# tjiiv-cprg/EPro-PnP

Hardware: AMD Instinct MI355X
Metric: PnP instances/sec (fwd+bwd, N=512 pts, 512 samples) (higher is better)
Workload: dtype f32; 1 GPU; C2 batched synthetic: 4096 objects/GPU x N=512 points, S=512 MC samples, K=4 AMIS iters, L=3 LM iters, EProPnP6DoF fwd+bwd; objects_per_gpu=4096, objects_total=4096, num_points=512, mc_samples=512, amis_iters=4, lm_iters=3, dof=6, parallelism=objects sharded x1, no data-path collective

## Files before the change

epro-pnp_amd/csrc/amis_common.h:

```cpp
#pragma once
#include "pnp_host.h"
#include "tuning.h"

namespace pnp {

typedef PNP_FIT_T fit_t;

__device__ __forceinline__ float sat_mul(float x, float one_v) {
  return __builtin_amdgcn_fmed3f(x * one_v, 0.0f, 1.0f);
}

__device__ __forceinline__ float sat_fma(float a, float b, float c) {
  return __builtin_amdgcn_fmed3f(fmaf(a, b, c), 0.0f, 1.0f);
}

__device__ __forceinline__ float clamp_below(float x, float lo) {
  int xi, li;
  memcpy(&xi, &x, 4);
  memcpy(&li, &lo, 4);
  const int mi = max(xi, li);
  float r;
  memcpy(&r, &mi, 4);
  return r;
}
// ... 58 lines not shown


PNP_FIT_FN void fit_translation(fit_t (&C)[3][3], const float* fallback_diag, float* rec) {
  fit_t invd[3];
  const bool ok = cholesky<3, fit_t>(C, invd);
  rec[37] = ok ? 0.f : 1.f;
  if (!ok) {
#pragma unroll
    for (int i = 0; i < 3; ++i) {
#pragma unroll
      for (int j = 0; j < 3; ++j) C[i][j] = (i == j) ? (fit_t)fallback_diag[i] : fit_t(0);
      invd[i] = fit_t(1) / (fit_t)fallback_diag[i];
    }
  }
  fit_t Li[3][3];
  tri_inverse<3, fit_t>(C, invd, Li);
  float sl = 0.f;
#pragma unroll
  for (int i = 0; i < 3; ++i) {
    sl += fast_log((float)C[i][i]);
#pragma unroll
    for (int j = 0; j <= i; ++j) {
      rec[3 + tri(i, j)] = (float)C[i][j];
      rec[9 + tri(i, j)] = (float)Li[i][j];
    }
  }
  rec[15] = student_t3_log_norm(sl);
}

constexpr int kRefitMaxVals = 21;
constexpr int kRefitRedFloats = kRefitMaxVals * kSumTRow + 24;
constexpr int kRefitHalfVals = 11;
constexpr int kRefitHalfFloats = kRefitHalfVals * kSumTRow + 24;

template <int NV, int ROWS = kRefitMaxVals>
PNP_FN void wave_sum_t(float (&v)[NV], float* lds, int lane) {
  static_assert(NV <= ROWS, "scratch rows");
  float* tot = lds + ROWS * kSumTRow;
#pragma unroll
  for (int i = 0; i < NV; ++i) lds[i * kSumTRow + lane] = v[i];
  wave_lds_fence();
#pragma unroll
  for (int base = 0; base < NV; base += 16) {
    const int row = base + (lane >> 2);
    float part = 0.f;
    if (row < NV) {
      const float4* r = reinterpret_cast<const float4*>(lds + row * kSumTRow + 16 * (lane & 3));
      const float4 a = r[0], b = r[1], c = r[2], d = r[3];
      part = (((a.x + a.y) + (a.z + a.w)) + ((b.x + b.y) + (b.z + b.w))) + (((c.x + c.y) + (c.z + c.w)) + ((d.x + d.y) + (d.z + d.w)));
    }
    part = quad_sum(part);
    if (row < NV && (lane & 3) == 0) tot[row] = part;
  }
  wave_lds_fence();
#pragma unroll
  for (int i = 0; i < NV; ++i) v[i] = tot[i];
  wave_lds_fence();
}

template <int NV, int ROWS = kRefitMaxVals>
PNP_FN void refit_sum(float (&v)[NV], float* scratch, int lane) {
  wave_sum_t<NV, ROWS>(v, scratch, lane);
}

template <int NV>
PNP_FN void wave_sum_fit(fit_t (&v)[NV], float* lds, int lane) {
  static_assert(NV <= 8 && NV * 64 * sizeof(fit_t) <= kRefitHalfFloats * sizeof(float), "one row of 64 per value, eight lanes per row");
  fit_t* row = reinterpret_cast<fit_t*>(lds);
#pragma unroll
  for (int i = 0; i < NV; ++i) row[i * 64 + lane] = v[i];
  wave_lds_fence();
  if (lane < 8 * NV) {
    fit_t* r = row + 8 * lane;
    r[0] = ((r[0] + r[1]) + (r[2] + r[3])) + ((r[4] + r[5]) + (r[6] + r[7]));
  }
  wave_lds_fence();
  if (lane < NV) {
    fit_t* r = row + 64 * lane;
    r[0] = ((r[0] + r[8]) + (r[16] + r[24])) + ((r[32] + r[40]) + (r[48] + r[56]));
  }
  wave_lds_fence();
#pragma unroll
  for (int i = 0; i < NV; ++i) v[i] = row[64 * i];
  wave_lds_fence();
}

PNP_FN void refit_translation_cov(const AmisParams& a, const float* smp, const float* lgw, int S, int M, float mx, float mu0, float mu1,
                                  float mu2, float invZ, float* scratch, int lane, fit_t (&C)[6]) {
  fit_t dl[3];
#pragma unroll
  for (int i = 0; i < 6; ++i) C[i] = fit_t(0);
#pragma unroll
  for (int i = 0; i < 3; ++i) dl[i] = fit_t(0);
  if (PNP_ABLATED(a, 8)) C[0] = C[2] = C[5] = fit_t(1);
  else
  for (int m = lane; m < M; m += 64) {
    const float e = fast_exp(lgw[m] - mx);
    const fit_t d0 = (fit_t)(smp[m] - mu0), d1 = (fit_t)(smp[S + m] - mu1), d2 = (fit_t)(smp[2 * S + m] - mu2);
    const fit_t e0 = (fit_t)e * d0, e1 = (fit_t)e * d1, e2 = (fit_t)e * d2;
    dl[0] += e0; dl[1] += e1; dl[2] += e2;
    C[0] += e0 * d0; C[1] += e1 * d0; C[2] += e1 * d1;
    C[3] += e2 * d0; C[4] += e2 * d1; C[5] += e2 * d2;
  }
  if (!PNP_ABLATED(a, 16)) {
    wave_sum_fit<6>(C, scratch, lane);
    wave_sum_fit<3>(dl, scratch, lane);
  }
  const fit_t iz = (fit_t)invZ;
#pragma unroll
  for (int i = 0; i < 3; ++i) dl[i] *= iz;
#pragma unroll
  for (int i = 0; i < 3; ++i)
#pragma unroll
    for (int j = 0; j <= i; ++j) C[tri(i, j)] = C[tri(i, j)] * iz - dl[i] * dl[j];
  const fit_t tol = fit_t(1e-12);
  const fit_t l21 = C[4] - C[3] * C[1] / C[0];
  const fit_t p1 = C[2] - C[1] * C[1] / C[0];
  const fit_t p2 = C[5] - C[3] * C[3] / C[0] - l21 * l21 / p1;
  if (p1 <= tol * C[2] || p2 <= tol * C[5]) C[0] = fit_t(NAN);
}

PNP_FIT_FN void fit_factor_pair(fit_t (&A)[4][4], int which, float dispersion, const float (&fallback)[4], float* rec) {
  const fit_t m01 = A[0][0] * A[1][1] - A[0][1] * A[1][0], m02 = A[0][0] * A[1][2] - A[0][2] * A[1][0],
               m03 = A[0][0] * A[1][3] - A[0][3] * A[1][0], m12 = A[0][1] * A[1][2] - A[0][2] * A[1][1],
               m13 = A[0][1] * A[1][3] - A[0][3] * A[1][1], m23 = A[0][2] * A[1][3] - A[0][3] * A[1][2];
  const fit_t n01 = A[2][0] * A[3][1] - A[2][1] * A[3][0], n02 = A[2][0] * A[3][2] - A[2][2] * A[3][0],
               n03 = A[2][0] * A[3][3] - A[2][3] * A[3][0], n12 = A[2][1] * A[3][2] - A[2][2] * A[3][1],
               n13 = A[2][1] * A[3][3] - A[2][3] * A[3][1], n23 = A[2][2] * A[3][3] - A[2][3] * A[3][2];
  const float det = (float)(m01 * n23 - m02 * n13 + m03 * n12 + m12 * n03 - m13 * n02 + m23 * n01);
  const fit_t add = (which == 0) ? (fit_t)(sqrtf(sqrtf(det)) * dispersion) : fit_t(0);
  fit_t invd[4];
#pragma unroll
  for (int i = 0; i < 4; ++i) A[i][i] += add;
  const bool ok = cholesky<4, fit_t>(A, invd) && (add == add);
  if (!ok) {
#pragma unroll
    for (int i = 0; i < 4; ++i) {
#pragma unroll
      for (int j = 0; j < 4; ++j) A[i][j] = (i == j) ? (fit_t)fallback[i] : fit_t(0);
// ... 185 lines not shown
    if (!done && (acc || a == kVmTries - 1)) {
      x = ((u3 - 0.5f >= 0.0f) ? 2.0f : -2.0f) * atan2f(srm1 * sh, srp1 * ch);
    }
    done = done || acc;
  }
  float y = x + loc + 3.14159265358979f;
  y = y - 6.283185307179586f * floorf(y * 0.15915494309189535f);
  return y - 3.14159265358979f;
}


template <int PL>
PNP_FN void store_pose(float* dst, const float (&ps)[PL]) {
  typedef float f4_a4 __attribute__((vector_size(16), aligned(4)));
  const f4_a4 head = {ps[0], ps[1], ps[2], ps[3]};
  *reinterpret_cast<f4_a4*>(dst) = head;
  if (PL == 7) {
    const f4_a4 tail = {ps[3], ps[PL > 4 ? 4 : 0], ps[PL > 5 ? 5 : 0], ps[PL > 6 ? 6 : 0]};
    *reinterpret_cast<f4_a4*>(dst + 3) = tail;
  }
}

struct AmisCtx {
  float* ptab;
  float* smp;
  float* cst;
  float* mixl;
  float* lgw;
  float* cpart;
  float* prop;
  float* red;
  float* nzb;
  float* rred;
  int S, K, s, T, tid, b;
  int cstride;
};

template <int DOF>
PNP_FN void base_noise(const AmisParams& a, int b, int m, float (&out)[8]) {
  const uint32_t k0 = (uint32_t)a.seed, k1 = (uint32_t)(a.seed >> 32);
  const uint32_t c2 = (uint32_t)a.offset, c3base = (uint32_t)(a.offset >> 32) * 64u;
  float nrm[12];
#pragma unroll
  for (int q = 0; q < (DOF == 6 ? 3 : 2); ++q) {
    const Philox4 r = philox4x32_10((uint32_t)b, (uint32_t)m, c2, c3base + q, k0, k1);
    box_muller(r.v[0], r.v[1], nrm[q * 4], nrm[q * 4 + 1]);
    box_muller(r.v[2], r.v[3], nrm[q * 4 + 2], nrm[q * 4 + 3]);
  }
  out[0] = nrm[0]; out[1] = nrm[1]; out[2] = nrm[2];
  out[3] = nrm[3] * nrm[3] + nrm[4] * nrm[4] + nrm[5] * nrm[5];
  if (DOF == 6) {
    out[4] = nrm[6]; out[5] = nrm[7]; out[6] = nrm[8]; out[7] = nrm[9];
  } else {
    out[4] = out[5] = out[6] = out[7] = 0.f;
  }
}

template <int DOF>
PNP_FN void amis_base_noise(const AmisCtx& cx, const AmisParams& a, int it, int first) {
  if (cx.nzb == nullptr || cx.tid < first) return;
  for (int n = cx.tid - first; n < cx.s; n += cx.T - first) {
    float nz8[8];
    base_noise<DOF>(a, cx.b, it * cx.s + n, nz8);
    reinterpret_cast<float4*>(cx.nzb)[2 * n] = make_float4(nz8[0], nz8[1], nz8[2], nz8[3]);
    reinterpret_cast<float4*>(cx.nzb)[2 * n + 1] = make_float4(nz8[4], nz8[5], nz8[6], nz8[7]);
  }
}

template <int DOF>
PNP_FN void amis_draw(const AmisCtx& cx, const Problem& p, const AmisParams& a, int it, const float (&Kc)[9],
                      const float* __restrict__ noise, float* __restrict__ pose_samples, int n0 = 0, int cnt = -1) {
  constexpr int PL = PoseLen<DOF>::value;
  constexpr int NZ = (DOF == 6) ? 8 : 4 + 3 * kVmTries;
  float* ptab = cx.ptab; float* smp = cx.smp;
  const int S = cx.S, K = cx.K, s = cx.s, T = cx.T, tid = cx.tid, b = cx.b;
  const float* rec = cx.prop + it * kPropStride;
  const bool nz_aliased = (cx.nzb != nullptr) && (cx.nzb == cx.ptab);
  float4 nz_a = make_float4(0.f, 0.f, 0.f, 0.f), nz_b = nz_a;
  if (nz_aliased) {
    if (tid < s) {
      nz_a = reinterpret_cast<const float4*>(cx.nzb)[2 * tid];
      nz_b = reinterpret_cast<const float4*>(cx.nzb)[2 * tid + 1];
    }
    __syncthreads();
  }
  const int n_end = (cnt < 0) ? s : n0 + cnt;
  for (int n = n0 + tid; n < n_end; n += T) {
    const int m = it * s + n;
    float z[3], chi2, g[4];
    if (noise != nullptr) {
      const float* nz = noise + (((size_t)b * K + it) * s + n) * NZ;
      z[0] = nz[0]; z[1] = nz[1]; z[2] = nz[2]; chi2 = nz[3];
      if (DOF == 6) {
        g[0] = nz[4]; g[1] = nz[5]; g[2] = nz[6]; g[3] = nz[7];
// ... 79 lines not shown
PNP_FN void amis_weights(const AmisCtx& cx, const AmisParams& a, int it, int WP) {
  constexpr int PL = PoseLen<DOF>::value;
  float* smp = cx.smp; float* cst = cx.cst; float* mixl = cx.mixl; float* lgw = cx.lgw; float* cpart = cx.cpart; float* prop = cx.prop;
  const int S = cx.S, s = cx.s, T = cx.T, tid = cx.tid;
  const float* rec = prop + it * kPropStride;
  const int M = (it + 1) * s;
  const float log_n = logf((float)(it + 1));
  for (int m = tid; m < M; m += T) {
    float ps[PL];
#pragma unroll
    for (int i = 0; i < PL; ++i) ps[i] = smp[i * S + m];
    float mix;
    if (m >= it * s) {
      if (WP > 0) {
        float c = cpart[m - it * s];
        for (int q = 1; q < WP; ++q) c += cpart[q * cx.cstride + (m - it * s)];
        cst[m] = c;
      }
      if (PNP_ABLATED(a, 4)) {
        mix = 0.f;
      } else {
        mix = proposal_logprob<DOF>(prop, ps);
        for (int j = 1; j <= it; ++j) mix = log_add_exp(mix, proposal_logprob<DOF>(prop + j * kPropStride, ps));
      }
    } else {
      mix = PNP_ABLATED(a, 4) ? 0.f : log_add_exp(mixl[m], proposal_logprob<DOF>(rec, ps));
    }
    mixl[m] = mix;
    lgw[m] = -cst[m] - (mix - log_n);
  }

}

template <int DOF, bool HALF = false>
PNP_FN void amis_refit(const AmisCtx& cx, const AmisParams& a, int it) {
  static_assert(!HALF || DOF == 6, "the half-size scratch serves the 6-DoF refit");
  constexpr int ROWS = HALF ? kRefitHalfVals : kRefitMaxVals;
  float* smp = cx.smp; float* lgw = cx.lgw; float* prop = cx.prop; float* red = cx.red;
  const int S = cx.S, s = cx.s;
  const float* rec = prop + it * kPropStride;
  const int M = (it + 1) * s;
  float* nrec = prop + (it + 1) * kPropStride;
  if (wave_id() != 0) {
    amis_base_noise<DOF>(cx, a, it + 1, 64);
    __syncthreads();
    return;
  }
  const int T = 64, tid = cx.tid;
  PNP_REFIT_BEGIN();
  if (PNP_ABLATED(a, 2)) {
    for (int i = tid; i < kPropStride; i += T) nrec[i] = rec[i];
    __syncthreads();
    return;
  }
  float mx = -INFINITY;
  for (int m = tid; m < M; m += T) mx = fmaxf(mx, lgw[m]);
  mx = wave_max(mx);
  const float p0 = rec[0], p1 = rec[1], p2 = rec[2];
  if (DOF == 6) {
    float mom[15];
#pragma unroll
    for (int i = 0; i < 15; ++i) mom[i] = 0.f;
    if (PNP_ABLATED(a, 8)) mom[0] = mom[4] = mom[6] = mom[9] = mom[13] = mom[14] = 1.f;
    else
    for (int m = tid; m < M; m += T) {
      const float e = fast_exp(lgw[m] - mx);
      const float d0 = smp[m] - p0, d1 = smp[S + m] - p1, d2 = smp[2 * S + m] - p2;
      mom[0] += e;
      mom[1] += e * d0; mom[2] += e * d1; mom[3] += e * d2;
// ... 50 lines not shown
          red[10 + i] = (float)invd[i];
#pragma unroll
          for (int j = 0; j < i; ++j) red[tri(i, j)] = (float)Sg[i][j];
        }
      }
      wave_lds_fence();
#pragma unroll
      for (int i = 0; i < 10; ++i) Lf[i] = red[i];
#pragma unroll
      for (int i = 0; i < 4; ++i) Ld[i] = red[10 + i];
      wave_lds_fence();
#pragma unroll
      for (int i = 0; i < 11; ++i) acc[i] = 0.f;
      for (int m = tid; m < M; m += T) {
        const float e = fast_exp(lgw[m] - mx);
        const float q0 = smp[3 * S + m], q1 = smp[4 * S + m], q2 = smp[5 * S + m], q3 = smp[6 * S + m];
        const float y0 = q0 * Ld[0];
        const float y1 = fmaf(-Lf[tri(1, 0)], y0, q1) * Ld[1];
        const float y2 = fmaf(-Lf[tri(2, 1)], y1, fmaf(-Lf[tri(2, 0)], y0, q2)) * Ld[2];
        const float y3 = fmaf(-Lf[tri(3, 2)], y2, fmaf(-Lf[tri(3, 1)], y1, fmaf(-Lf[tri(3, 0)], y0, q3))) * Ld[3];
        const float Mq = fmaf(y3, y3, fmaf(y2, y2, fmaf(y1, y1, y0 * y0)));
        const float iw = e * fast_rcp(fmaxf(Mq, a.eps));
        acc[10] += iw;
        acc[0] += iw * q0 * q0;
        acc[1] += iw * q1 * q0; acc[2] += iw * q1 * q1;
        acc[3] += iw * q2 * q0; acc[4] += iw * q2 * q1; acc[5] += iw * q2 * q2;
        acc[6] += iw * q3 * q0; acc[7] += iw * q3 * q1; acc[8] += iw * q3 * q2; acc[9] += iw * q3 * q3;
      }
      refit_sum<11, ROWS>(acc, cx.rred, tid);
    }
    PNP_REFIT_PHASE(1);
    if (tid < 2) {
      if (tid == 0) {
        nrec[0] = mu0; nrec[1] = mu1; nrec[2] = mu2;
        nrec[39] = 0.f;
      }
      fit_t A4[4][4];
      const fit_t inorm = (a.mle_iter > 0) ? fit_t(1) / (fit_t)acc[10] : fit_t(0);
#pragma unroll
      for (int i = 0; i < 4; ++i)
#pragma unroll
        for (int j = 0; j <= i; ++j) {
          fit_t v = (a.mle_iter > 0) ? (fit_t)acc[tri(i, j)] * inorm + ((i == j) ? (fit_t)a.eps : fit_t(0))
                                      : ((i == j) ? fit_t(1) : fit_t(0));
          if (tid == 1) v = (i < 3) ? c6[tri(i, j)] : ((i == j) ? fit_t(1) : fit_t(0));
          A4[i][j] = v;
          A4[j][i] = v;
        }
      const float dflt[4] = {1.f, 1.f, 1.f, 1.f};
      fit_factor_pair(A4, tid, a.dispersion, dflt, nrec);
    }
    PNP_REFIT_PHASE(2);
  } else {
    float mom[6];
#pragma unroll
    for (int i = 0; i < 6; ++i) mom[i] = 0.f;
    for (int m = tid; m < M; m += T) {
      const float e = fast_exp(lgw[m] - mx);
      const float d0 = smp[m] - p0, d1 = smp[S + m] - p1, d2 = smp[2 * S + m] - p2;
      mom[0] += e;
      mom[1] += e * d0; mom[2] += e * d1; mom[3] += e * d2;
      const float yaw = smp[3 * S + m];
      float sy, cy;
      sincos_rad(yaw, sy, cy);
      mom[4] += e * sy;
      mom[5] += e * cy;
    }
// ... 34 lines not shown
```

epro-pnp_amd/csrc/amis_forward_mfma.hip:

```cpp
#include "amis_common.h"
#include "dispatch.h"

namespace pnp {



template <bool BOUNDS, bool FOLDED = false>
__device__ __forceinline__ void huber_cost_4(const floatx4& hx, const floatx4& hy, const floatx4& hz, const float4& w4,
                                             float zmin_v, float one_v, const Bounds& bd, f32x2 (&acc2)[2]) {
  static_assert(!(BOUNDS && FOLDED), "the clamp acts on the un-weighted projection");
  const f32x2 wu2 = {w4.x, w4.x}, wv2 = {w4.y, w4.y}, cu2 = {w4.z, w4.z}, cv2 = {w4.w, w4.w};
  const f32x2 mhalf = {-0.5f, -0.5f};
#pragma unroll
  for (int h = 0; h < 2; ++h) {
    const float z0 = clamp_below(hz[2 * h], zmin_v), z1 = clamp_below(hz[2 * h + 1], zmin_v);
    const f32x2 rz2 = {fast_rcp(z0), fast_rcp(z1)};
    const f32x2 hx2 = {hx[2 * h], hx[2 * h + 1]}, hy2 = {hy[2 * h], hy[2 * h + 1]};
    f32x2 rx2, ry2;
    if (FOLDED) {
      rx2 = fma2(hx2, rz2, cu2);
      ry2 = fma2(hy2, rz2, cv2);
    } else {
      f32x2 px2 = hx2 * rz2, py2 = hy2 * rz2;
      if (BOUNDS) {
        px2 = f32x2{clamp_lu(px2[0], bd.lbx, bd.ubx), clamp_lu(px2[1], bd.lbx, bd.ubx)};
        py2 = f32x2{clamp_lu(py2[0], bd.lby, bd.uby), clamp_lu(py2[1], bd.lby, bd.uby)};
      }
      rx2 = fma2(px2, wu2, cu2);
      ry2 = fma2(py2, wv2, cv2);
    }
    const f32x2 s2 = fma2(rx2, rx2, ry2 * ry2);
    const f32x2 rho2 = {fast_sqrt(s2[0]), fast_sqrt(s2[1])};
    const f32x2 m2 = {sat_mul(rho2[0], one_v), sat_mul(rho2[1], one_v)};
    acc2[h] = fma2(m2, fma2(mhalf, m2, rho2), acc2[h]);
  }
}

constexpr int kChunk = 1024;

struct MfmaShape {
  int chunk;
  int s16;
  int ahead;
  int chunks;
};

template <int DOF, bool BOUNDS, int NPT, bool SPILL = false, bool SPLIT = false, bool BF16 = false, bool CHUNKED = false, bool WLDS = false>
__global__ __launch_bounds__(512, SPLIT ? 2 : (DOF == 6 ? (NPT <= 8 ? (BF16 ? (WLDS ? PNP_FWD_WLDS_MINW : PNP_FWD_BF16_MINW) : PNP_FWD_MINW) : 2) : (NPT <= 2 ? 3 : 2))) void amis_forward_mfma_kernel(Problem p, AmisParams a_in, MfmaShape sh,
                                                                  const float* __restrict__ pose_opt,
                                                                  const float* __restrict__ pose_cov,
                                                                  const float* __restrict__ noise,
                                                                  float* __restrict__ pose_samples,
                                                                  float* __restrict__ logweights,
                                                                  float* __restrict__ proposals,
                                                                  float* __restrict__ spill, int nsplit,
                                                                  float* __restrict__ xch) {
  static_assert(!SPILL || NPT == 0, "the spill variant streams the points");
  static_assert(!SPLIT || NPT > 0, "the split over workgroups is a register-mode variant");
  static_assert(!WLDS || (BF16 && DOF == 6 && NPT > 0 && !SPLIT && !CHUNKED && !SPILL), "weights in LDS: the one-workgroup bf16 6-DoF kernel");
  constexpr int PL = PoseLen<DOF>::value;
  const int G = SPLIT ? nsplit : 1;
  static_assert(!CHUNKED || (NPT > 0 && !SPLIT && !SPILL), "chunks are a register-mode variant of the one-workgroup kernel");
  const int CH = CHUNKED ? sh.chunks : 1;
  const int GT = SPLIT ? G : CH;
  int b, part = 0;
  if (SPLIT) {
    const int g = (int)blockIdx.x, per = (p.B + 7) >> 3, idx = g >> 3;
    part = idx % G;
    b = (g & 7) * per + idx / G;
  } else {
    b = object_of_block(p.B);
  }
  if (b >= p.B) return;
  AmisParams a = a_in;
  if (a.offset_dev != nullptr) a.offset += *a.offset_dev;
  const int T = (int)blockDim.x, tid = (int)threadIdx.x, lane = lane_id(), wv = wave_id(), W = T >> 6;
  const int S = a.S, K = a.K, s = S / K, s16 = sh.s16, NC = sh.chunk;

  PNP_PHASES_BEGIN(6);
  PNP_DYN_SMEM(float, smem);
  constexpr bool kRegs = NPT > 0;
  static_assert(!BF16 || NPT > 0, "the split projection is a register-mode variant");
  constexpr bool kBf = BF16;
  typedef ProjOp<kBf> Proj;
  constexpr bool kFold = kRegs && !BOUNDS && !kBf;
  const int WPs = kRegs ? (G > 1 ? G : W) : 1;
  const int cpart_rows = kRegs ? (SPLIT ? W + G : W) : 1;
  float* ptab = smem;
  float* pB = ptab + 12 * s16;
  float* pW = pB + 4 * NC;
  float* smp = SPILL ? spill + (size_t)b * (PL + 3) * S : pW + 4 * NC;
  float* cst = smp + PL * S;
  float* mixl = cst + S;
  float* lgw = mixl + S;
  float* cpart = SPILL ? pW + 4 * NC : smp + (((PL + 3) * S + 3) & ~3);
  float* gath = cpart + W * s16;
  float* prop = cpart + (WLDS ? max(cpart_rows * s16, kRefitHalfFloats) : cpart_rows * s16) + (SPLIT ? 4 : 0);
  float* red = prop + K * kPropStride;
  float* wl = red + 256;
  float* rred = WLDS ? cpart : red + 256;
  float* nzb = (s <= T) ? ptab : (WLDS ? wl + W * NPT * 64 : rred + kRefitRedFloats);

  float Kc[9], delta;
  Bounds bd;
  load_camera<BOUNDS>(p, b, Kc, bd, delta);
  const float zmin_v = to_vgpr(p.z_min), one_v = to_vgpr(1.0f);
  const HuberScale hs = huber_scale(delta);
  const float inv_delta = hs.inv_delta, delta_sq = hs.delta_sq;

  const bool tiled = SPILL && s > s16;
  AmisCtx cx;
  cx.ptab = ptab; cx.smp = smp; cx.cst = cst; cx.mixl = mixl; cx.lgw = lgw; cx.cpart = SPLIT ? gath : cpart; cx.prop = prop; cx.red = red;
  cx.S = S; cx.K = K; cx.s = s; cx.T = T; cx.tid = tid; cx.b = b; cx.cstride = s16;
  cx.nzb = (noise == nullptr && W > 1 && sh.ahead) ? nzb : nullptr;
  cx.rred = rred;

  if (!tiled)
    for (int i = tid; i < 12 * (s16 - s); i += T) ptab[12 * s + i] = 0.f;
  if (tid < (DOF == 6 ? 2 : 1))
    initial_fit<DOF>(pose_opt + (size_t)b * PL, pose_cov + (size_t)b * DOF * DOF, a.eps, a.dispersion, prop, tid);
  if (part == 0 && tid == T - 1) denormalise_pose_opt<DOF>(a, pose_opt, b);
  const int nchunk = kRegs ? 1 : (p.N + NC - 1) / NC;
  auto load_chunk = [&](int c0) {
    const int cnt = min(NC, ((p.N - c0 + 15) >> 4) << 4);
    for (int n = tid; n < cnt; n += T) {
      const Point q = load_point(p, b, c0 + n);
      reinterpret_cast<float4*>(pB)[n] = make_float4(q.X, q.Y, q.Z, 1.0f);
      const float wu = q.wu * inv_delta, wv = q.wv * inv_delta;
      reinterpret_cast<float4*>(pW)[n] = make_float4(wu, wv, -q.u * wu, -q.v * wv);
    }
  };
  typename Proj::T rB[kRegs ? NPT : 1];
  float4 rW[kRegs ? NPT : 1];
  auto load_tiles = [&](int pt) {
#pragma unroll
    for (int i = 0; i < (kRegs ? NPT : 1); ++i) {
      const Point q = load_point(p, b, ((pt * W + wv) + GT * W * i) * 16 + (lane & 15));
      const int k4 = lane >> 4;
      const int wslot = (wv * NPT + i) * 16 + (lane & 15);
      const float bval = (k4 == 0) ? q.X : (k4 == 1) ? q.Y : (k4 == 2) ? q.Z : 1.0f;
      rB[i] = Proj::b(bval);
      const float wu = q.wu * inv_delta, wv = q.wv * inv_delta;
      if constexpr (WLDS) {
        if (k4 == 0) reinterpret_cast<float4*>(wl)[wslot] = make_float4(wu, wv, -q.u * wu, -q.v * wv);
      } else {
        rW[i] = kFold ? make_float4(bval * wu, bval * wv, -q.u * wu, -q.v * wv) : make_float4(wu, wv, -q.u * wu, -q.v * wv);
      }
    }
// ... 142 lines not shown
        const unsigned v = xwg_poll(slot + q * s16 + m, (((miss | gone_parts) >> q) & 1u) ? 0u : a.split_timeout);
        if (v == kXwgEmpty) miss |= 1u << q; else gath[q * s16 + m] = bits_f32(v);
      }
      if (miss) atomicOr(reinterpret_cast<int*>(missw), (int)miss);
      __syncthreads();
      unsigned todo = *missw;
      gone_parts |= todo;
      if (todo) {
        if (tid == 0) raise_status(p, EPROPNP_ST_SPLIT_TIMEOUT, b);
        for (int q = 0; q < G; ++q) {
          if (!((todo >> q) & 1u)) continue;
          load_tiles(q);
          sweep_regs();
          __syncthreads();
          for (int m = tid; m < s; m += T) {
            float c = cpart[m];
            for (int w = 1; w < W; ++w) c += cpart[w * s16 + m];
            gath[q * s16 + m] = bits_f32(xwg_payload(c));
          }
          __syncthreads();
        }
        load_tiles(part);
      }
    }
    PNP_PHASE(2);

    if (tiled) __syncthreads();
    AmisCtx cxw = cx;
    cxw.tid = (int)f32_bits(to_vgpr(bits_f32((unsigned)tid)));
    amis_weights<DOF>(cxw, a, it, tiled ? 0 : WPs);
    __syncthreads();
    PNP_PHASE(3);
    if (it == K - 1) break;
    amis_refit<DOF, WLDS>(cxw, a, it);
    PNP_PHASE(4);
  }

  if (part == 0) {
    int st_bits = 0;
    for (int m = tid; m < S; m += T) {
      const float lw = lgw[m];
      logweights[(size_t)m * p.B + b] = lw;
      if (a.sample_costs != nullptr) a.sample_costs[(size_t)m * p.B + b] = cst[m];
      st_bits |= (lw == lw && lw != INFINITY) ? 0 : EPROPNP_ST_NONFINITE_WEIGHT;
    }
    for (int i = tid; i < K; i += T)
      st_bits |= (prop[i * kPropStride + 37] != 0.f || prop[i * kPropStride + 38] != 0.f) ? EPROPNP_ST_CHOL_FALLBACK : 0;
    raise_status(p, st_bits, b);
  }
  if (proposals != nullptr && part == 0)
    for (int i = tid; i < K * kPropStride; i += T) proposals[(size_t)b * K * kPropStride + i] = prop[i];
  PNP_PHASE(5);
  advance_counters(a, p.B * G);
  PNP_PHASES_FLUSH(6);
}

int tuning_phase_cycles(unsigned long long* out, int reset) { return tuning::read_cycles(out, reset, true); }

template <class F>
static int dispatch_npt(int npt, F&& f) {
  switch (npt) {
    case 0: return f(ic<0>{});
    case 1: return f(ic<1>{});
    case 2: return f(ic<2>{});
    case 4: return f(ic<4>{});
    case 8: return f(ic<8>{});
    case 12: return f(ic<12>{});
    default: return f(ic<16>{});
  }
}

static int forward_split_parts(int B, int ptiles) {
  const long wgs = padded_object_grid(B), cus = device_cu_count();
  int g = 8;
  while (g > 1 && (wgs * g > cus || 8 * g > ptiles)) g >>= 1;
  if (g < 4) g = 1;
  { int ov[1]; if (env_ints("EPROPNP_FWD_SPLIT", ov, 1) && (ov[0] == 1 || ov[0] == 2 || ov[0] == 4 || ov[0] == 8) && wgs * ov[0] <= 4096 && 4 * ov[0] <= ptiles) g = ov[0]; }
  return g;
}

unsigned long long amis_forward_split_bytes(const epropnp_problem* prob, int mc_samples, int num_iter) {
  if (prob == nullptr || prob->num_obj <= 0 || num_iter <= 0 || mc_samples % num_iter != 0) return 0;
  const int ptiles = (prob->num_pts + 15) / 16;
  const int g = forward_split_parts(prob->num_obj, ptiles);
  if (g <= 1 || (ptiles + 4 * g - 1) / (4 * g) > 8) return 0;
  const int s16 = ((mc_samples / num_iter + 15) / 16) * 16;
  return sizeof(float) * (unsigned long long)prob->num_obj * num_iter * g * s16;
}

struct FwdPlan {
  MfmaShape sh;
  int waves, npt, G;
  size_t smem;
  bool bf16, spilled, truncated, chunked;
  bool wlds;
};

constexpr size_t kLdsPerCu = 160 * 1024, kLdsGranule = 1280;

static int plan_amis_forward(const epropnp_problem* prob, int S, int K, unsigned long long scratch_bytes, FwdPlan* out) {
  const int B = prob->num_obj, N = prob->num_pts;
  const int s = S / K;
  const int PL = prob->dof == 6 ? 7 : 4;
  MfmaShape& sh = out->sh;
  sh.s16 = ((s + 15) / 16) * 16;
  const int ptiles = (N + 15) / 16;
  const int npt_opts[6] = {1, 2, 4, 8, 12, 16};
  int waves = 4, npt = 0, best = 1 << 30;
  for (int w : {4, 8, 2, 1}) {
    for (int o : npt_opts) {
      if (w * o >= ptiles && w * o < best) { best = w * o; waves = w; npt = o; }
      if (w * o >= ptiles) break;
    }
  }
  if (prob->dof == 4 && npt >= 12) npt = 0;
  if (B < 512 && waves == 4 && npt == 8) { waves = 8; npt = 4; }
  { int ov[2]; if (tune_ints("fwd_mfma", ov, 2) && (ov[0] == 1 || ov[0] == 2 || ov[0] == 4 || ov[0] == 8) && (ov[1] == 0 || ov[1] == 1 || ov[1] == 2 || ov[1] == 4 || ov[1] == 8 || ov[1] == 12 || ov[1] == 16) && (ov[1] == 0 || ov[0] * ov[1] >= ptiles)) { waves = ov[0]; npt = ov[1]; } }
  if (npt == 0) {
    sh.chunk = ((N + 15) / 16) * 16;
    if (sh.chunk > kChunk) sh.chunk = kChunk;
    if (best == (1 << 30)) waves = 4;
    const int tiles = sh.s16 / 16;
    while (waves > 1 && waves > tiles) waves /= 2;
  } else {
    sh.chunk = 0;
  }
  int G = 1;
  {
    const int g = forward_split_parts(B, ptiles);
// ... 29 lines not shown
    spilled = true;
    waves = 8; npt = 0; G = 1; sh.chunks = 1;
    sh.chunk = ((N + 15) / 16) * 16;
    if (sh.chunk > kChunk) sh.chunk = kChunk;
    const int tiles = sh.s16 / 16;
    while (waves > 1 && waves > tiles) waves /= 2;
    smem = lds_bytes(true);
    if (smem > 160 * 1024) {
      sh.ahead = 0;
      const size_t fixed = sizeof(float) * (8 * (size_t)sh.chunk + (size_t)K * kPropStride + 256 + kRefitRedFloats);
      const size_t rows = (160 * 1024 - fixed) / (sizeof(float) * 13);
      if ((size_t)sh.s16 > rows) sh.s16 = (int)(rows / 16) * 16;
      if (sh.s16 < 16) return fail(EPROPNP_EINVAL, "amis_forward: no LDS left for a pose tile (%d points per chunk)", sh.chunk);
      smem = lds_bytes(true);
    }
  }
  bool bf16 = npt >= 1;
  if (const char* e = getenv("EPROPNP_FWD_PROJ")) bf16 = (e[0] == 'f') ? false : bf16;
  out->waves = waves; out->npt = npt; out->G = G; out->smem = smem;
  out->bf16 = bf16; out->spilled = spilled; out->truncated = sh.s16 < s16_full;
  out->chunked = !spilled && G == 1 && npt == 8 && (sh.chunks > 1 || (bf16 && tune_flag("fwd_chunked")));
  out->wlds = false;
  if (prob->dof == 6 && bf16 && !spilled && !out->chunked && G == 1 && waves == 4 && npt == 8) {
    const size_t smem_w = lds_bytes(false, true);
    const size_t granules = (smem_w + kLdsGranule - 1) / kLdsGranule * kLdsGranule;
    bool take = 4 * granules <= kLdsPerCu && (long)padded_object_grid(B) > 3L * device_cu_count();
    { int ov[1]; if (tune_ints("fwd_wlds", ov, 1)) take = ov[0] != 0 && smem_w <= kLdsPerCu; }
    if (take) { out->wlds = true; out->smem = smem_w; }
    if (take && PNP_FWD_WLDS_MINW < 4) {
      const size_t hold = kLdsPerCu / PNP_FWD_WLDS_MINW / kLdsGranule * kLdsGranule;
      if (out->smem < hold) out->smem = hold;
    }
  }
  return EPROPNP_OK;
}

int plan_amis_forward_record(const epropnp_problem* prob, int S, int K, unsigned long long scratch_bytes, int32_t* out) {
  FwdPlan plan;
  if (int rc = plan_amis_forward(prob, S, K, scratch_bytes, &plan)) return rc;
  out[0] = plan.waves; out[1] = plan.npt; out[2] = plan.G; out[3] = plan.sh.chunks; out[4] = plan.bf16; out[5] = plan.spilled;
  out[6] = plan.truncated; out[7] = plan.chunked;
  return EPROPNP_OK;
}

int launch_amis_forward(const epropnp_problem* prob, const epropnp_amis_params* am, const float* pose_opt,
                        const float* pose_cov, const float* noise, float* pose_samples, float* logweights,
                        float* proposals, hipStream_t st, const DenormOut* dn, float* sample_costs) {
  if (int rc = check_problem(prob)) return rc;
  if (!am) return fail(EPROPNP_EINVAL, "amis_forward: params NULL");
  if (am->num_iter <= 0 || am->mc_samples <= 0 || am->mc_samples % am->num_iter != 0)
    return fail(EPROPNP_EINVAL, "amis_forward: mc_samples (%d) must be a positive multiple of num_iter (%d)",
                am->mc_samples, am->num_iter);
  if (prob->num_obj == 0) return EPROPNP_OK;
  if (!pose_opt || !pose_cov || !pose_samples || !logweights) return fail(EPROPNP_EINVAL, "amis_forward: NULL pointer");
  const Problem d = to_device_problem(prob);
  const int S = am->mc_samples, K = am->num_iter;
  const int PL = prob->dof == 6 ? 7 : 4;
  FwdPlan plan;
  if (int rc = plan_amis_forward(prob, S, K, am->split_scratch != nullptr ? am->split_scratch_bytes : 0, &plan)) return rc;
  const MfmaShape sh = plan.sh;
  const int waves = plan.waves, npt = plan.npt, G = plan.G;
  const size_t smem = plan.smem;
  const bool bf16 = plan.bf16;
  AmisParams k;
  k.S = S; k.K = K; k.unused_wp = 1; k.eps = am->eps; k.mle_iter = am->acg_mle_iter; k.dispersion = am->acg_dispersion;
  k.seed = am->seed; k.offset = am->offset; k.offset_dev = (const unsigned long long*)am->offset_dev; k.ablate = 0;
  k.advance = (am->advance && am->advance_ticket && am->advance_count > 0) ? (unsigned long long*)am->advance : nullptr;
  k.advance_ticket = (int*)am->advance_ticket; k.advance_count = am->advance_count;
  k.split_timeout = split_timeout_cycles();
  k.dn_offset = dn ? dn->offset : nullptr; k.dn_samples = dn ? dn->samples : nullptr; k.dn_pose_opt = dn ? dn->pose_opt : nullptr;
  k.sample_costs = sample_costs;
  { int ab[1]; if (tune_ints("ablate", ab, 1)) k.ablate = ab[0]; }
  float* spill = nullptr;
  if (plan.spilled &&
      hipMallocAsync((void**)&spill, sizeof(float) * (size_t)(PL + 3) * S * d.B, st) != hipSuccess) {
    (void)hipGetLastError();
    return fail(EPROPNP_ELAUNCH, "amis_forward: mc_samples %d needs a %zu B scratch buffer and hipMallocAsync failed "
                "(stream capture?)", S, sizeof(float) * (size_t)(PL + 3) * S * d.B);
  }
  const dim3 grid(padded_object_grid(d.B)), block(64 * waves);
  if (spill != nullptr) {
    dispatch_dof_bounds(prob->dof, has_bounds(prob), [&](auto DOF, auto BND) -> int {
      auto kern = amis_forward_mfma_kernel<decltype(DOF)::value, decltype(BND)::value, 0, true>;
      allow_dynamic_lds((const void*)kern, smem);
      PNP_LAUNCH(kern, grid, block, smem, st, d, k, sh, pose_opt, pose_cov, noise, pose_samples, logweights, proposals, spill, 1,
                 (float*)nullptr);
      return 0;
    });
    const int rc = check_launch("amis_forward_mfma_kernel (sampler state in global scratch)");
    (void)hipFreeAsync(spill, st);
    return rc;
  }
  float* xch = nullptr;
  char* owned = nullptr;
  dim3 grid_split = grid;
  if (G > 1) {
    const size_t xbytes = sizeof(float) * (size_t)d.B * K * G * sh.s16;
    char* mem = (am->split_scratch != nullptr && am->split_scratch_bytes >= xbytes) ? (char*)am->split_scratch : nullptr;
    if (mem == nullptr) {
      if (hipMallocAsync((void**)&mem, xbytes, st) != hipSuccess) {
        (void)hipGetLastError();
        return fail(EPROPNP_ELAUNCH, "amis_forward: scratch for the %d-way split (%zu B) could not be allocated", G, xbytes);
      }
      owned = mem;
    }
    if (!exchange_prefilled(mem, xbytes) &&
        launch_fill_u32(mem, 0xffffffffu, xbytes / 4, st) != EPROPNP_OK) {
      (void)hipGetLastError();
      return fail(EPROPNP_ELAUNCH, "amis_forward: could not fill the split scratch");
    }
    xch = (float*)mem;
    grid_split = dim3(padded_object_grid(d.B) * G);
  }
  if (G > 1) {
    dispatch_dof_bounds(prob->dof, has_bounds(prob), [&](auto DOF, auto BND) -> int {
      auto go = [&](auto NPT) -> int {
        auto run = [&](auto kern) -> int {
          allow_dynamic_lds((const void*)kern, smem);
          PNP_LAUNCH(kern, grid_split, block, smem, st, d, k, sh, pose_opt, pose_cov, noise, pose_samples, logweights, proposals,
                     (float*)nullptr, G, xch);
          return 0;
        };
        if (bf16) return run(amis_forward_mfma_kernel<decltype(DOF)::value, decltype(BND)::value, decltype(NPT)::value, false, true, true>);
        return run(amis_forward_mfma_kernel<decltype(DOF)::value, decltype(BND)::value, decltype(NPT)::value, false, true>);
      };
      switch (npt) {
        case 1: return go(ic<1>{});
        case 2: return go(ic<2>{});
        case 4: return go(ic<4>{});
        default: return go(ic<8>{});
      }
    });
  } else {
    dispatch_dof_bounds(prob->dof, has_bounds(prob), [&](auto DOF, auto BND) -> int {
      return dispatch_npt(npt, [&](auto NPT) -> int {
        auto run = [&](auto kern) -> int {
          allow_dynamic_lds((const void*)kern, smem);
          PNP_LAUNCH(kern, grid, block, smem, st, d, k, sh, pose_opt, pose_cov, noise, pose_samples, logweights, proposals,
                     (float*)nullptr, 1, (float*)nullptr);
          return 0;
        };
        if constexpr (decltype(NPT)::value == 8) {
          if (plan.chunked)
            return run(amis_forward_mfma_kernel<decltype(DOF)::value, decltype(BND)::value, 8, false, false, true, true>);
          if constexpr (decltype(DOF)::value == 6) {
            if (plan.wlds)
              return run(amis_forward_mfma_kernel<6, decltype(BND)::value, 8, false, false, true, false, true>);
          }
        }
        if constexpr (decltype(NPT)::value >= 1) {
          if (bf16) return run(amis_forward_mfma_kernel<decltype(DOF)::value, decltype(BND)::value, decltype(NPT)::value, false, false, true>);
        }
        return run(amis_forward_mfma_kernel<decltype(DOF)::value, decltype(BND)::value, decltype(NPT)::value>);
      });
    });
  }
  if (owned != nullptr) (void)hipFreeAsync(owned, st);
  return check_launch("amis_forward_mfma_kernel");
}

}
```

Baseline: 3.036 million instances/s.

## Split 6-DoF AMIS refit across two waves for rotation and translation fits

Adds a two-wave refit path for the 6-DoF AMIS forward kernel. Wave 0 fits the rotation ACG covariance while the last wave fits the translation mean and covariance in a separate LDS scratch, and the middle waves generate the next iteration's base noise. Previously a single refit sequence handled both fits. The aim is to shorten the serial refit phase between AMIS iterations by running the two fits concurrently. In exchange it needs extra LDS scratch, carefully placed alongside the weight table when weights live in LDS, more kernel template instantiations, and NaN canonicalisation of the mean outputs.

```diff
diff --git a/epro-pnp_amd/csrc/amis_common.h b/epro-pnp_amd/csrc/amis_common.h
--- a/epro-pnp_amd/csrc/amis_common.h
+++ b/epro-pnp_amd/csrc/amis_common.h
@@ -114,6 +114,9 @@
 constexpr int kRefitRedFloats = kRefitMaxVals * kSumTRow + 24;
 constexpr int kRefitHalfVals = 11;
 constexpr int kRefitHalfFloats = kRefitHalfVals * kSumTRow + 24;
+constexpr int kFitSplitVals = 3;
+constexpr int kFitSplitFloats = (4 * kSumTRow + 24) > kFitSplitVals * 64 * (int)(sizeof(fit_t) / sizeof(float))
+                                    ? (4 * kSumTRow + 24) : kFitSplitVals * 64 * (int)(sizeof(fit_t) / sizeof(float));
 
 template <int NV, int ROWS = kRefitMaxVals>
 PNP_FN void wave_sum_t(float (&v)[NV], float* lds, int lane) {
@@ -145,9 +148,9 @@
   wave_sum_t<NV, ROWS>(v, scratch, lane);
 }
 
-template <int NV>
+template <int NV, int FLOATS = kRefitHalfFloats>
 PNP_FN void wave_sum_fit(fit_t (&v)[NV], float* lds, int lane) {
-  static_assert(NV <= 8 && NV * 64 * sizeof(fit_t) <= kRefitHalfFloats * sizeof(float), "one row of 64 per value, eight lanes per row");
+  static_assert(NV <= 8 && NV * 64 * sizeof(fit_t) <= FLOATS * sizeof(float), "one row of 64 per value, eight lanes per row");
   fit_t* row = reinterpret_cast<fit_t*>(lds);
 #pragma unroll
   for (int i = 0; i < NV; ++i) row[i * 64 + lane] = v[i];
@@ -167,6 +170,7 @@
   wave_lds_fence();
 }
 
+template <bool BY3 = false>
 PNP_FN void refit_translation_cov(const AmisParams& a, const float* smp, const float* lgw, int S, int M, float mx, float mu0, float mu1,
                                   float mu2, float invZ, float* scratch, int lane, fit_t (&C)[6]) {
   fit_t dl[3];
@@ -185,8 +189,17 @@
     C[3] += e2 * d0; C[4] += e2 * d1; C[5] += e2 * d2;
   }
   if (!PNP_ABLATED(a, 16)) {
-    wave_sum_fit<6>(C, scratch, lane);
-    wave_sum_fit<3>(dl, scratch, lane);
+    if constexpr (BY3) {
+      fit_t c0[3] = {C[0], C[1], C[2]}, c1[3] = {C[3], C[4], C[5]};
+      wave_sum_fit<3, kFitSplitFloats>(c0, scratch, lane);
+      wave_sum_fit<3, kFitSplitFloats>(c1, scratch, lane);
+      wave_sum_fit<3, kFitSplitFloats>(dl, scratch, lane);
+#pragma unroll
+      for (int i = 0; i < 3; ++i) { C[i] = c0[i]; C[3 + i] = c1[i]; }
+    } else {
+      wave_sum_fit<6>(C, scratch, lane);
+      wave_sum_fit<3>(dl, scratch, lane);
+    }
   }
   const fit_t iz = (fit_t)invZ;
 #pragma unroll
@@ -438,6 +451,8 @@
   float* red;
   float* nzb;
   float* rred;
+  float* tfit;
+  int tfit_off;
   int S, K, s, T, tid, b;
   int cstride;
 };
@@ -463,9 +478,10 @@
 }
 
 template <int DOF>
-PNP_FN void amis_base_noise(const AmisCtx& cx, const AmisParams& a, int it, int first) {
-  if (cx.nzb == nullptr || cx.tid < first) return;
-  for (int n = cx.tid - first; n < cx.s; n += cx.T - first) {
+PNP_FN void amis_base_noise(const AmisCtx& cx, const AmisParams& a, int it, int first, int end = -1) {
+  if (end < 0) end = cx.T;
+  if (cx.nzb == nullptr || cx.tid < first || cx.tid >= end) return;
+  for (int n = cx.tid - first; n < cx.s; n += end - first) {
     float nz8[8];
     base_noise<DOF>(a, cx.b, it * cx.s + n, nz8);
     reinterpret_cast<float4*>(cx.nzb)[2 * n] = make_float4(nz8[0], nz8[1], nz8[2], nz8[3]);
@@ -611,9 +627,159 @@
 
 }
 
-template <int DOF, bool HALF = false>
+PNP_FN float canonical_nan(float x) { return (x != x) ? bits_f32(0x7fc00000u) : x; }
+
+template <bool HALF>
+PNP_FN void amis_refit_two(const AmisCtx& cx, const AmisParams& a, int it) {
+  constexpr int ROWS = HALF ? kRefitHalfVals : kRefitMaxVals;
+  float* smp = cx.smp; float* lgw = cx.lgw; float* prop = cx.prop; float* red = cx.red;
+  const int S = cx.S, s = cx.s, W = cx.T >> 6, wv = wave_id();
+  const float* rec = prop + it * kPropStride;
+  const int M = (it + 1) * s;
+  float* nrec = prop + (it + 1) * kPropStride;
+  const bool rot = wv == 0, tra = wv == W - 1;
+  if (!rot) amis_base_noise<6>(cx, a, it + 1, 64, W >= 3 ? cx.T - 64 : cx.T);
+  if (!rot && !tra) {
+    __syncthreads();
+    return;
+  }
+  const int T = 64, tid = cx.tid, lane = tid & 63;
+  PNP_REFIT_BEGIN();
+  if (PNP_ABLATED(a, 2)) {
+    if (rot) for (int i = lane; i < kPropStride; i += T) nrec[i] = rec[i];
+    __syncthreads();
+    return;
+  }
+  float mx = -INFINITY;
+  for (int m = lane; m < M; m += T) mx = fmaxf(mx, lgw[m]);
+  mx = wave_max(mx);
+  fit_t A4[4][4];
+  if (rot) {
+    float acc[11];
+#pragma unroll
+    for (int i = 0; i < 11; ++i) acc[i] = 0.f;
+    if (PNP_ABLATED(a, 8)) acc[0] = acc[2] = acc[5] = acc[9] = acc[10] = 1.f;
+    else
+    for (int m = lane; m < M; m += T) {
+      const float e = fast_exp(lgw[m] - mx);
+      const float q0 = smp[3 * S + m], q1 = smp[4 * S + m], q2 = smp[5 * S + m], q3 = smp[6 * S + m];
+      const float iw = e * fast_rcp(fmaxf(q0 * q0 + q1 * q1 + q2 * q2 + q3 * q3, a.eps));
+      acc[0] += iw * q0 * q0;
+      acc[1] += iw * q1 * q0; acc[2] += iw * q1 * q1;
+      acc[3] += iw * q2 * q0; acc[4] += iw * q2 * q1; acc[5] += iw * q2 * q2;
+      acc[6] += iw * q3 * q0; acc[7] += iw * q3 * q1; acc[8] += iw * q3 * q2; acc[9] += iw * q3 * q3;
+      acc[10] += iw;
+    }
+    if (!PNP_ABLATED(a, 16)) refit_sum<11, ROWS>(acc, cx.rred, lane);
+    PNP_REFIT_PHASE(0);
+    float Lf[10], Ld[4];
+    for (int r = 1; r < a.mle_iter; ++r) {
+      if (lane == 0) {
+        fit_t Sg[4][4], invd[4];
+        const fit_t inorm = fit_t(1) / (fit_t)acc[10];
+#pragma unroll
+        for (int i = 0; i < 4; ++i)
+#pragma unroll
+          for (int j = 0; j <= i; ++j) {
+            const fit_t v = (fit_t)acc[tri(i, j)] * inorm + ((i == j) ? (fit_t)a.eps : fit_t(0));
+            Sg[i][j] = v;
+            Sg[j][i] = v;
+          }
+        cholesky<4, fit_t>(Sg, invd);
+#pragma unroll
+        for (int i = 0; i < 4; ++i) {
+          red[10 + i] = (float)invd[i];
+#pragma unroll
+          for (int j = 0; j < i; ++j) red[tri(i, j)] = (float)Sg[i][j];
+        }
+      }
+      wave_lds_fence();
+#pragma unroll
+      for (int i = 0; i < 10; ++i) Lf[i] = red[i];
+#pragma unroll
+      for (int i = 0; i < 4; ++i) Ld[i] = red[10 + i];
+      wave_lds_fence();
+#pragma unroll
+      for (int i = 0; i < 11; ++i) acc[i] = 0.f;
+      for (int m = lane; m < M; m += T) {
+        const float e = fast_exp(lgw[m] - mx);
+        const float q0 = smp[3 * S + m], q1 = smp[4 * S + m], q2 = smp[5 * S + m], q3 = smp[6 * S + m];
+        const float y0 = q0 * Ld[0];
+        const float y1 = fmaf(-Lf[tri(1, 0)], y0, q1) * Ld[1];
+        const float y2 = fmaf(-Lf[tri(2, 1)], y1, fmaf(-Lf[tri(2, 0)], y0, q2)) * Ld[2];
+        const float y3 = fmaf(-Lf[tri(3, 2)], y2, fmaf(-Lf[tri(3, 1)], y1, fmaf(-Lf[tri(3, 0)], y0, q3))) * Ld[3];
+        const float Mq = fmaf(y3, y3, fmaf(y2, y2, fmaf(y1, y1, y0 * y0)));
+        const float iw = e * fast_rcp(fmaxf(Mq, a.eps));
+        acc[10] += iw;
+        acc[0] += iw * q0 * q0;
+        acc[1] += iw * q1 * q0; acc[2] += iw * q1 * q1;
+        acc[3] += iw * q2 * q0; acc[4] += iw * q2 * q1; acc[5] += iw * q2 * q2;
+        acc[6] += iw * q3 * q0; acc[7] += iw * q3 * q1; acc[8] += iw * q3 * q2; acc[9] += iw * q3 * q3;
+      }
+      refit_sum<11, ROWS>(acc, cx.rred, lane);
+    }
+    PNP_REFIT_PHASE(1);
+    if (lane == 0) nrec[39] = 0.f;
+    const fit_t inorm = (a.mle_iter > 0) ? fit_t(1) / (fit_t)acc[10] : fit_t(0);
+#pragma unroll
+    for (int i = 0; i < 4; ++i)
+#pragma unroll
+      for (int j = 0; j <= i; ++j) {
+        const fit_t v = (a.mle_iter > 0) ? (fit_t)acc[tri(i, j)] * inorm + ((i == j) ? (fit_t)a.eps : fit_t(0))
+                                          : ((i == j) ? fit_t(1) : fit_t(0));
+        A4[i][j] = v;
+        A4[j][i] = v;
+      }
+  } else {
+    const float p0 = rec[0], p1 = rec[1], p2 = rec[2];
+    float mom[4] = {0.f, 0.f, 0.f, 0.f};
+    if (PNP_ABLATED(a, 8)) mom[0] = 1.f;
+    else
+    for (int m = lane; m < M; m += T) {
+      const float e = fast_exp(lgw[m] - mx);
+      const float d0 = smp[m] - p0, d1 = smp[S + m] - p1, d2 = smp[2 * S + m] - p2;
+      mom[0] += e;
+      mom[1] += e * d0; mom[2] += e * d1; mom[3] += e * d2;
+    }
+    if (!PNP_ABLATED(a, 16)) refit_sum<4, 4>(mom, cx.tfit, lane);
+    const float invZ = 1.0f / mom[0];
+    const float dl0 = mom[1] * invZ, dl1 = mom[2] * invZ, dl2 = mom[3] * invZ;
+    const float mu0 = p0 + dl0, mu1 = p1 + dl1, mu2 = p2 + dl2;
+    fit_t c6[6];
+    refit_translation_cov<true>(a, smp, lgw, S, M, mx, mu0, mu1, mu2, invZ, cx.tfit, lane, c6);
+    if (lane == 0) {
+      nrec[0] = canonical_nan(mu0); nrec[1] = canonical_nan(mu1); nrec[2] = canonical_nan(mu2);
+    }
+#pragma unroll
+    for (int i = 0; i < 4; ++i)
+#pragma unroll
+      for (int j = 0; j <= i; ++j) {
+        const fit_t v = (i < 3) ? c6[tri(i, j)] : ((i == j) ? fit_t(1) : fit_t(0));
+        A4[i][j] = v;
+        A4[j][i] = v;
+      }
+    const int pad0 = 12 * s, pad1 = 12 * cx.cstride, off = cx.tfit_off;
+    if (off >= 0 && off < pad1 && off + kFitSplitFloats > pad0)
+      for (int i = off + lane; i < min(off + kFitSplitFloats, pad1); i += T)
+        if (i >= pad0) cx.ptab[i] = 0.f;
+  }
+  if (lane == 0) {
+    const int which = (int)f32_bits(to_vgpr(bits_f32(rot ? 0u : 1u)));
+    const float dflt[4] = {1.f, 1.f, 1.f, 1.f};
+    fit_factor_pair(A4, which, a.dispersion, dflt, nrec);
+  }
+  PNP_REFIT_PHASE(2);
+  __syncthreads();
+}
+
+template <int DOF, bool HALF = false, bool TWO = false>
 PNP_FN void amis_refit(const AmisCtx& cx, const AmisParams& a, int it) {
   static_assert(!HALF || DOF == 6, "the half-size scratch serves the 6-DoF refit");
+  static_assert(!TWO || DOF == 6, "two fitting waves: the 6-DoF refit");
+  if constexpr (TWO) {
+    amis_refit_two<HALF>(cx, a, it);
+    return;
+  }
   constexpr int ROWS = HALF ? kRefitHalfVals : kRefitMaxVals;
   float* smp = cx.smp; float* lgw = cx.lgw; float* prop = cx.prop; float* red = cx.red;
   const int S = cx.S, s = cx.s;
@@ -730,7 +896,7 @@
     PNP_REFIT_PHASE(1);
     if (tid < 2) {
       if (tid == 0) {
-        nrec[0] = mu0; nrec[1] = mu1; nrec[2] = mu2;
+        nrec[0] = canonical_nan(mu0); nrec[1] = canonical_nan(mu1); nrec[2] = canonical_nan(mu2);
         nrec[39] = 0.f;
       }
       fit_t A4[4][4];
diff --git a/epro-pnp_amd/csrc/amis_forward_mfma.hip b/epro-pnp_amd/csrc/amis_forward_mfma.hip
--- a/epro-pnp_amd/csrc/amis_forward_mfma.hip
+++ b/epro-pnp_amd/csrc/amis_forward_mfma.hip
@@ -43,9 +43,10 @@
   int s16;
   int ahead;
   int chunks;
+  int fit;
 };
 
-template <int DOF, bool BOUNDS, int NPT, bool SPILL = false, bool SPLIT = false, bool BF16 = false, bool CHUNKED = false, bool WLDS = false>
+template <int DOF, bool BOUNDS, int NPT, bool SPILL = false, bool SPLIT = false, bool BF16 = false, bool CHUNKED = false, bool WLDS = false, bool FIT2 = false>
 __global__ __launch_bounds__(512, SPLIT ? 2 : (DOF == 6 ? (NPT <= 8 ? (BF16 ? (WLDS ? PNP_FWD_WLDS_MINW : PNP_FWD_BF16_MINW) : PNP_FWD_MINW) : 2) : (NPT <= 2 ? 3 : 2))) void amis_forward_mfma_kernel(Problem p, AmisParams a_in, MfmaShape sh,
                                                                   const float* __restrict__ pose_opt,
                                                                   const float* __restrict__ pose_cov,
@@ -57,6 +58,7 @@
                                                                   float* __restrict__ xch) {
   static_assert(!SPILL || NPT == 0, "the spill variant streams the points");
   static_assert(!SPLIT || NPT > 0, "the split over workgroups is a register-mode variant");
+  static_assert(!FIT2 || DOF == 6, "two fitting waves: the 6-DoF refit");
   static_assert(!WLDS || (BF16 && DOF == 6 && NPT > 0 && !SPLIT && !CHUNKED && !SPILL), "weights in LDS: the one-workgroup bf16 6-DoF kernel");
   constexpr int PL = PoseLen<DOF>::value;
   const int G = SPLIT ? nsplit : 1;
@@ -114,6 +116,11 @@
   cx.S = S; cx.K = K; cx.s = s; cx.T = T; cx.tid = tid; cx.b = b; cx.cstride = s16;
   cx.nzb = (noise == nullptr && W > 1 && sh.ahead) ? nzb : nullptr;
   cx.rred = rred;
+  cx.tfit = nullptr; cx.tfit_off = -1;
+  if constexpr (FIT2) {
+    cx.tfit = WLDS ? ptab + sh.fit : rred + kRefitHalfVals * kSumTRow;
+    cx.tfit_off = WLDS ? sh.fit : -1;
+  }
 
   if (!tiled)
     for (int i = tid; i < 12 * (s16 - s); i += T) ptab[12 * s + i] = 0.f;
@@ -322,7 +329,7 @@
     __syncthreads();
     PNP_PHASE(3);
     if (it == K - 1) break;
-    amis_refit<DOF, WLDS>(cxw, a, it);
+    amis_refit<DOF, WLDS, FIT2>(cxw, a, it);
     PNP_PHASE(4);
   }
 
@@ -346,6 +353,14 @@
 }
 
 int tuning_phase_cycles(unsigned long long* out, int reset) { return tuning::read_cycles(out, reset, true); }
+
+template <int DOF, bool BOUNDS, int NPT, bool SPILL = false, bool SPLIT = false, bool BF16 = false, bool CHUNKED = false, bool WLDS = false>
+static auto forward_kernel(bool fit2) {
+  if constexpr (DOF == 6) {
+    if (fit2) return amis_forward_mfma_kernel<DOF, BOUNDS, NPT, SPILL, SPLIT, BF16, CHUNKED, WLDS, true>;
+  }
+  return amis_forward_mfma_kernel<DOF, BOUNDS, NPT, SPILL, SPLIT, BF16, CHUNKED, WLDS, false>;
+}
 
 template <class F>
 static int dispatch_npt(int npt, F&& f) {
@@ -385,6 +400,8 @@
   bool bf16, spilled, truncated, chunked;
   bool wlds;
 };
+
+static_assert(kRefitHalfVals * kSumTRow + kFitSplitFloats <= kRefitMaxVals * kSumTRow, "the second fitting wave's scratch: rows 11..20 of the refit's");
 
 constexpr size_t kLdsPerCu = 160 * 1024, kLdsGranule = 1280;
 
@@ -480,6 +497,13 @@
       if (out->smem < hold) out->smem = hold;
     }
   }
+  sh.fit = -1;
+  if (prob->dof == 6 && waves >= 2) {
+    const int off = !out->wlds ? 0 : (s <= 64 * waves ? 8 * s : 0);
+    if (!out->wlds || 12 * sh.s16 - off >= kFitSplitFloats) sh.fit = off;
+    int ov[1];
+    if (tune_ints("fwd_fit_split", ov, 1) && ov[0] == 0) sh.fit = -1;
+  }
   return EPROPNP_OK;
 }
 
@@ -509,7 +533,7 @@
   const MfmaShape sh = plan.sh;
   const int waves = plan.waves, npt = plan.npt, G = plan.G;
   const size_t smem = plan.smem;
-  const bool bf16 = plan.bf16;
+  const bool bf16 = plan.bf16, fit2 = sh.fit >= 0;
   AmisParams k;
   k.S = S; k.K = K; k.unused_wp = 1; k.eps = am->eps; k.mle_iter = am->acg_mle_iter; k.dispersion = am->acg_dispersion;
   k.seed = am->seed; k.offset = am->offset; k.offset_dev = (const unsigned long long*)am->offset_dev; k.ablate = 0;
@@ -529,7 +553,7 @@
   const dim3 grid(padded_object_grid(d.B)), block(64 * waves);
   if (spill != nullptr) {
     dispatch_dof_bounds(prob->dof, has_bounds(prob), [&](auto DOF, auto BND) -> int {
-      auto kern = amis_forward_mfma_kernel<decltype(DOF)::value, decltype(BND)::value, 0, true>;
+      auto kern = forward_kernel<decltype(DOF)::value, decltype(BND)::value, 0, true>(fit2);
       allow_dynamic_lds((const void*)kern, smem);
       PNP_LAUNCH(kern, grid, block, smem, st, d, k, sh, pose_opt, pose_cov, noise, pose_samples, logweights, proposals, spill, 1,
                  (float*)nullptr);
@@ -569,8 +593,8 @@
                      (float*)nullptr, G, xch);
           return 0;
         };
-        if (bf16) return run(amis_forward_mfma_kernel<decltype(DOF)::value, decltype(BND)::value, decltype(NPT)::value, false, true, true>);
-        return run(amis_forward_mfma_kernel<decltype(DOF)::value, decltype(BND)::value, decltype(NPT)::value, false, true>);
+        if (bf16) return run(forward_kernel<decltype(DOF)::value, decltype(BND)::value, decltype(NPT)::value, false, true, true>(fit2));
+        return run(forward_kernel<decltype(DOF)::value, decltype(BND)::value, decltype(NPT)::value, false, true>(fit2));
       };
       switch (npt) {
         case 1: return go(ic<1>{});
@@ -590,16 +614,16 @@
         };
         if constexpr (decltype(NPT)::value == 8) {
           if (plan.chunked)
-            return run(amis_forward_mfma_kernel<decltype(DOF)::value, decltype(BND)::value, 8, false, false, true, true>);
+            return run(forward_kernel<decltype(DOF)::value, decltype(BND)::value, 8, false, false, true, true>(fit2));
           if constexpr (decltype(DOF)::value == 6) {
             if (plan.wlds)
-              return run(amis_forward_mfma_kernel<6, decltype(BND)::value, 8, false, false, true, false, true>);
+              return run(forward_kernel<6, decltype(BND)::value, 8, false, false, true, false, true>(fit2));
           }
         }
         if constexpr (decltype(NPT)::value >= 1) {
-          if (bf16) return run(amis_forward_mfma_kernel<decltype(DOF)::value, decltype(BND)::value, decltype(NPT)::value, false, false, true>);
-        }
-        return run(amis_forward_mfma_kernel<decltype(DOF)::value, decltype(BND)::value, decltype(NPT)::value>);
+          if (bf16) return run(forward_kernel<decltype(DOF)::value, decltype(BND)::value, decltype(NPT)::value, false, false, true>(fit2));
+        }
+        return run(forward_kernel<decltype(DOF)::value, decltype(BND)::value, decltype(NPT)::value>(fit2));
       });
     });
   }
```

New measurement: 3.055 million instances/s (median of 6 runs). Within noise of the previous version (+0.6%).
